# mandt-lab/vbq

Measured on AMD Instinct MI355X. Metric: quantized latents/sec (32-lambda sweep; one count per (element, lambda) pair and entropy-model build), higher is better.
Workload: dtype f32; 1 GPU; kodak24_c256 [36864 x 256] f32, 32-lambda sweep, N=10; step = two-pass entropy-model build (quantizer.py:82-150); elements_per_gpu=9437184, lambdas=32, parallelism=element-sharded x1, launch=one HIP graph replay per step

## Files before the change

### vbq_amd/csrc/vbq_quantize_fast.hip

```cpp
#include <stddef.h>

#include "vbq_common.h"
#include "vbq_sweep.h"

namespace vbq {
namespace {

constexpr int kFastThreads = 256;
#ifndef VBQ_FAST_NE
#define VBQ_FAST_NE 2
#endif
#ifndef VBQ_FAST_WAVES
#define VBQ_FAST_WAVES 4
#endif
#ifndef VBQ_SLOW_INLINE
#define VBQ_SLOW_INLINE __noinline__
#endif
constexpr int kFastNE = VBQ_FAST_NE;

__device__ __forceinline__ float dist_cost(float P, float mu, double rinv) {
    const float d = __fsub_rn(P, mu);
    const float t = (float)__dmul_rn((double)d, rinv);
    const float q = __fmul_rn(t, t);
    return __fmul_rn(0.5f, q);
}

__device__ __forceinline__ float min3f(float a, float b, float c) { return fminf(fminf(a, b), c); }

template <bool NT>
__device__ __forceinline__ void store_idx2(uint32_t *p, uint32_t v) {
    if constexpr (NT) __builtin_nontemporal_store(v, p);
    else *p = v;
}

template <int M>
__device__ __forceinline__ float min_of(const float (&v)[M]) {
    float t[M];
#pragma unroll
    for (int i = 0; i < M; ++i) t[i] = v[i];
    int m = M;
#pragma unroll
    for (int pass = 0; pass < 8; ++pass) {
        if (m <= 1) break;
        int o = 0;
        int i = 0;
#pragma unroll
        for (; i + 2 < m; i += 3) t[o++] = min3f(t[i], t[i + 1], t[i + 2]);
        if (o == 0) { t[o++] = fminf(t[0], t[1]); i = 2; }
        for (; i < m; ++i) t[o++] = t[i];
        m = o;
    }
    return t[0];
}

template <int N>
struct LevelInfo {
    float dL, dR;
    uint32_t posL, posR;
};

template <int N>
__device__ __forceinline__ LevelInfo<N> descend(const float *tb, int n, float z, double sg, uint32_t &g) {
    const int off = (1 << n) - 1;
    const int m = 1 << n;
    const uint32_t j = g;
    const float pj = tb[off + j];
    const bool below = pj < z;
    LevelInfo<N> r;
    if (n == 0) {
        r.dL = r.dR = dist_cost(pj, z, sg);
        r.posL = r.posR = 0;
    } else {
        int jo = below ? (int)j + 1 : (int)j - 1;
        jo = jo < 0 ? 0 : (jo > m - 1 ? m - 1 : jo);
        bool swap = false;
        if (n == N && below && j == (uint32_t)(m - 1)) { jo = m - 2; swap = true; }
        const float po = tb[off + jo];
        const float dj = dist_cost(pj, z, sg);
        const float dn = dist_cost(po, z, sg);
        const bool j_is_left = below && !swap;
        r.dL = j_is_left ? dj : dn;
        r.dR = j_is_left ? dn : dj;
        r.posL = j_is_left ? j : (uint32_t)jo;
        r.posR = j_is_left ? (uint32_t)jo : j;
    }
    g = 2 * g + (below ? 1u : 0u);
    return r;
}

template <int N>
__device__ VBQ_SLOW_INLINE uint32_t exact_rank_scan(const float *tb, float z, float sigma, const float *pen) {
    const double sg = __ddiv_rn(1.0, (double)sigma);
    uint32_t g = 0;
    float bestL = 0.f, bestR = 0.f;
    uint32_t rkL = 0, rkR = 0;
    for (int n = 0; n <= N; ++n) {
        const LevelInfo<N> li = descend<N>(tb, n, z, sg, g);
        const float p = pen[n];
        const float cL = __fadd_rn(li.dL, p);
        if (n == 0 || cL < bestL) { bestL = cL; rkL = ((2 * li.posL + 1) << (N - n)) - 1; }
        if (n >= 1) {
            const float cR = __fadd_rn(li.dR, p);
            if (n == 1 || cR < bestR) { bestR = cR; rkR = ((2 * li.posR + 1) << (N - n)) - 1; }
        }
    }
    if (N == 0) return rkL;
    return (bestL <= bestR) ? rkL : rkR;
}

template <int N, int MODE>
__global__ void __launch_bounds__(kFastThreads, VBQ_FAST_WAVES)
k_quant_fast(const float *__restrict__ mu, const float *__restrict__ sg, long n_per_ch, long ch_stride, int C,
             const float *__restrict__ table, Lambdas32 lam, const float *__restrict__ len,
             int L, uint16_t *__restrict__ out_idx, float *__restrict__ out_zhat,
             float *__restrict__ out_bits, long E, int vec_ok, int dbg,
             unsigned long long *__restrict__ level_counts) {
    constexpr int T = table_size(N);
    constexpr int N1 = N + 1;
    constexpr int NE = kFastNE;
    constexpr bool EXTRA = MODE == 1;
    constexpr bool COUNT = MODE == 2;
    const bool never_flag = dbg == 2;
    constexpr int PS = (N1 + 3) & ~3;
    __shared__ float tb[T + 1];
    __shared__ uint32_t scratch[N1 * NE * kFastThreads];
    __shared__ __align__(16) float penl[kMaxLambdaChunk * PS];
    const int c = blockIdx.y;
    if (COUNT) {
        for (int i = threadIdx.x; i < N1 * NE * kFastThreads; i += blockDim.x) scratch[i] = 0;
    }
    for (int i = threadIdx.x; i < T; i += blockDim.x) tb[i] = table[(long)c * T + i];
    int odd = 0;
    for (int i = threadIdx.x; i < L * PS; i += blockDim.x) {
        const int l = i / PS, n = i - l * PS;
        const float p = n < N1 ? __fmul_rn(lam.lam[l], len ? len[((long)l * C + c) * N1 + n] : (float)n) : 0.0f;
        penl[i] = p;
        odd |= (len != nullptr && !(p == 0.0f || (p >= 1.8189894e-12f && p <= 1.1805916e21f))) ? 1 : 0;
    }
    const bool force_slow = dbg == 1 || __syncthreads_or(odd) != 0;

    const long base = (long)c * ch_stride;
    const long nquads = (n_per_ch + NE - 1) / NE;

    auto load_group = [&](long q, float (&m)[NE], float (&sv)[NE]) {
        const long i0 = q * NE;
        if (!(vec_ok & 2) && (vec_ok & 1) && (i0 + NE <= n_per_ch)) {
            if constexpr (NE == 4) {
                const float4 mv = *reinterpret_cast<const float4 *>(mu + base + i0);
                const float4 s4v = *reinterpret_cast<const float4 *>(sg + base + i0);
                m[0] = mv.x; m[1] = mv.y; m[2] = mv.z; m[3] = mv.w;
                sv[0] = s4v.x; sv[1] = s4v.y; sv[2] = s4v.z; sv[3] = s4v.w;
            } else {
                const float2 mv = *reinterpret_cast<const float2 *>(mu + base + i0);
                const float2 s2v = *reinterpret_cast<const float2 *>(sg + base + i0);
                m[0] = mv.x; m[1] = mv.y;
                sv[0] = s2v.x; sv[1] = s2v.y;
            }
        } else {
#pragma unroll
            for (int k = 0; k < NE; ++k) {
                const bool ok = i0 + k < n_per_ch;
                const long at = (vec_ok & 2) ? (i0 + k) * C + c : base + i0 + k;
                m[k] = ok ? mu[at] : 0.0f;
                sv[k] = ok ? sg[at] : 1.0f;
            }
        }
    };
    const long q0 = (long)blockIdx.x * blockDim.x + threadIdx.x, qstep = (long)gridDim.x * blockDim.x;
    float mn[NE], sn[NE];
#pragma unroll
    for (int k = 0; k < NE; ++k) { mn[k] = 0.0f; sn[k] = 1.0f; }
    if (q0 < nquads) load_group(q0, mn, sn);
    const bool resident = (vec_ok & 4) != 0;
    unsigned int rot = wave_slot();
    for (long q = q0; q < nquads; q += qstep) {
        if (resident) __builtin_amdgcn_s_setprio(3);
        const long i0 = q * NE;
        const bool full = (vec_ok & 1) && (i0 + NE <= n_per_ch);
        float m4[NE], s4[NE];
#pragma unroll
        for (int k = 0; k < NE; ++k) { m4[k] = mn[k]; s4[k] = sn[k]; }
        {
            const long qn = q + qstep < nquads ? q + qstep : q;
            load_group(qn, mn, sn);
        }

        float du[NE][N1];
        uint32_t g[NE];
        double rinv[NE];
#pragma unroll
        for (int k = 0; k < NE; ++k) {
            g[k] = 0;
            rinv[k] = __ddiv_rn(1.0, (double)s4[k]);
        }
        const char *tbb = reinterpret_cast<const char *>(tb);
#pragma unroll
        for (int n = 0; n <= N; ++n) {
            constexpr int kWordMask = 0xffe00000u;
            const int off4 = 4 * ((1 << n) - 1);
            const int top4 = 4 * ((1 << n) - 1);
#pragma unroll
            for (int k = 0; k < NE; ++k) {
                const float pj = *reinterpret_cast<const float *>(tbb + off4 + g[k]);
                const bool below = pj < m4[k];
                float dL, dR;
                uint32_t lo4, hi4;
                if (n == 0) {
                    dL = dR = dist_cost(pj, m4[k], rinv[k]);
                    lo4 = hi4 = 0;
                } else {
                    const uint32_t G4 = g[k] + (below ? 4u : 0u);
                    int lo = (int)G4 - 4;
                    lo = lo < 0 ? 0 : lo;
                    if (n == N) lo = lo > top4 - 4 ? top4 - 4 : lo;
                    lo4 = (uint32_t)lo;
                    hi4 = G4 > (uint32_t)top4 ? (uint32_t)top4 : G4;
                    dL = dist_cost(*reinterpret_cast<const float *>(tbb + off4 + lo4), m4[k], rinv[k]);
                    dR = dist_cost(*reinterpret_cast<const float *>(tbb + off4 + hi4), m4[k], rinv[k]);
                }
                du[k][n] = vmin(dL, dR);
                g[k] = 2 * g[k] + (below ? 4u : 0u);
                if (COUNT) continue;
                const bool r_better = dR < dL;
                const uint32_t b4 = r_better ? hi4 : lo4;
                const uint32_t better = n < N ? (b4 << (N - n - 1)) + ((1u << (N - n)) - 1u) : (b4 >> 1);
                const uint32_t gap = __float_as_uint(__fsub_rn(dR, dL)) ^ 0x80000000u;
                scratch[(n * NE + k) * kFastThreads + threadIdx.x] = (gap & kWordMask) | better;
            }
        }

        if (resident) {
            set_issue_priority(rot);
            rot += 3u;
        }
        for (int l = 0; l < L; ++l) {
            const float *pp = penl + l * PS;
            float p[N1];
#pragma unroll
            for (int n = 0; n < N1; ++n) p[n] = pp[n];
            uint32_t rank[NE];
            float cst[NE][N1];
            float S[NE];
            uint32_t ne[NE];
#pragma unroll
            for (int n = 0; n < N1; ++n)
#pragma unroll
                for (int k = 0; k < NE; ++k) cst[k][n] = __fadd_rn(du[k][n], p[n]);
#pragma unroll
            for (int k = 0; k < NE; ++k) S[k] = min_of<N1>(cst[k]);
            {
#pragma unroll
                for (int k = 0; k < NE; ++k) ne[k] = 0;
#pragma unroll
                for (int n = N; n >= 0; --n)
#pragma unroll
                    for (int k = 0; k < NE; ++k)
                        ne[k] = __builtin_amdgcn_alignbit(ne[k], __float_as_uint(__fsub_rn(S[k], cst[k][n])), 31);
            }
            uint64_t fmk[NE];
            if constexpr (COUNT) {
                uint64_t any_multi = 0;
                uint32_t lvl[NE];
#pragma unroll
                for (int k = 0; k < NE; ++k) {
                    lvl[k] = (uint32_t)__builtin_ctz(~ne[k]);
                    const uint64_t multi = __builtin_amdgcn_uicmp((uint32_t)__popc(ne[k]), (uint32_t)N, 33);
                    fmk[k] = never_flag ? 0ull : (force_slow ? ~0ull : multi);
                    any_multi |= fmk[k];
                }
                if (any_multi != 0) {
                    const uint32_t lane = __lane_id();
#pragma unroll
                    for (int k = 0; k < NE; ++k)
                        if ((fmk[k] >> lane) & 1ull)
                            lvl[k] = (uint32_t)N - (uint32_t)__builtin_ctz(exact_rank_scan<N>(tb, m4[k], s4[k], pp) + 1u);
                }
                const uint32_t lane = threadIdx.x & 63u;
                const uint32_t inc = (lane & 16u) ? 0x10000u : 1u;
#pragma unroll
                for (int k = 0; k < NE; ++k)
                    if (i0 + k < n_per_ch) atomicAdd(&scratch[((uint32_t)(l * N1) + lvl[k]) * 16u + (lane & 15u)], inc);
                continue;
            }
            uint32_t pk[NE];
#pragma unroll
            for (int k = 0; k < NE; ++k) {
                const int n1 = __builtin_ctz(~ne[k]);
                pk[k] = scratch[(n1 * NE + k) * kFastThreads + threadIdx.x];
            }
            uint64_t fm[NE];
#pragma unroll
            for (int k = 0; k < NE; ++k) {
                const uint64_t multi = __builtin_amdgcn_uicmp((uint32_t)__popc(ne[k]), (uint32_t)N, 33);
                const uint32_t thr = __float_as_uint(__fmul_rn(S[k], 1.9073486328125e-06f));
                const uint64_t lr_close = __builtin_amdgcn_uicmp(pk[k], thr, 37);
                rank[k] = pk[k] & ((2u << N) - 1u);
                fm[k] = never_flag ? 0ull : (force_slow ? ~0ull : (multi | lr_close));
            }
            uint64_t any_flag = 0;
#pragma unroll
            for (int k = 0; k < NE; ++k) any_flag |= fm[k];
            if (any_flag != 0) {
                const uint32_t lane = __lane_id();
#pragma unroll
                for (int k = 0; k < NE; ++k)
                    if ((fm[k] >> lane) & 1ull) rank[k] = exact_rank_scan<N>(tb, m4[k], s4[k], pp);
            }
            const long o = (long)l * E + base + i0;
            float zh[NE], bt[NE];
            if (EXTRA) {
#pragma unroll
                for (int k = 0; k < NE; ++k) {
                    const uint32_t kk = rank[k] + 1;
                    const int tz = __builtin_ctz(kk);
                    const int lvl = N - tz;
                    const uint32_t pos = kk >> (tz + 1);
                    zh[k] = tb[(1 << lvl) - 1 + pos];
                    bt[k] = len ? len[((long)l * C + c) * N1 + lvl] : (float)lvl;
                }
            }
            if (full) {
                if constexpr (NE == 4) {
                    uint2 pk2;
                    pk2.x = rank[0] | (rank[1] << 16);
                    pk2.y = rank[2] | (rank[3] << 16);
                    *reinterpret_cast<uint2 *>(out_idx + o) = pk2;
                    if (EXTRA) {
                        if (out_zhat) *reinterpret_cast<float4 *>(out_zhat + o) = make_float4(zh[0], zh[1], zh[2], zh[3]);
                        if (out_bits) *reinterpret_cast<float4 *>(out_bits + o) = make_float4(bt[0], bt[1], bt[2], bt[3]);
                    }
                } else {
                    store_idx2<false>(reinterpret_cast<uint32_t *>(out_idx + o), rank[0] | (rank[1] << 16));
                    if (EXTRA) {
                        if (out_zhat) *reinterpret_cast<float2 *>(out_zhat + o) = make_float2(zh[0], zh[1]);
                        if (out_bits) *reinterpret_cast<float2 *>(out_bits + o) = make_float2(bt[0], bt[1]);
                    }
                }
            } else {
#pragma unroll
                for (int k = 0; k < NE; ++k) {
                    if (i0 + k < n_per_ch) {
                        out_idx[o + k] = (uint16_t)rank[k];
                        if (EXTRA) {
                            if (out_zhat) out_zhat[o + k] = zh[k];
                            if (out_bits) out_bits[o + k] = bt[k];
                        }
                    }
                }
            }
        }
    }
    if constexpr (COUNT) {
        __syncthreads();
        for (int i = threadIdx.x; i < L * N1; i += blockDim.x) {
            unsigned int v = 0;
#pragma unroll
            for (int j = 0; j < 16; ++j) {
                const unsigned int w = scratch[i * 16 + j];
                v += (w & 0xffffu) + (w >> 16);
            }
            const int l = i / N1, n = i - l * N1;
            if (v) atomicAdd(&level_counts[((long)l * C + c) * N1 + n], (unsigned long long)v);
        }
    }
}


#ifndef VBQ_HULL_WAVES
#define VBQ_HULL_WAVES 4
#endif
#ifndef VBQ_HULL_NE
#define VBQ_HULL_NE 2
#endif
#ifndef VBQ_HULL_THREADS
#define VBQ_HULL_THREADS 256
#endif
constexpr int kHullThreads = VBQ_HULL_THREADS;
#ifndef VBQ_HULL_COPIES
#define VBQ_HULL_COPIES 16
#endif
constexpr int kHullKeys = 2048;
constexpr int kFixQueue = 192;
struct HullSweep : SweepTable<32, kHullKeys> {};
static_assert(sizeof(HullSweep) == 2220 && offsetof(HullSweep, val) == 0 && offsetof(HullSweep, perm) == 128 && offsetof(HullSweep, L) == 160 &&
              offsetof(HullSweep, key0) == 164 && offsetof(HullSweep, nkeys) == 168 && offsetof(HullSweep, lut) == 172,
              "HullSweep travels in the kernel arguments: its layout is fixed");

template <int N>
__device__ __forceinline__ void hull_du_nearest(const char *tbb, float z, float sigma, float (&du)[N + 1]) {
    uint32_t g = 0;
    const double rinv = __ddiv_rn(1.0, (double)sigma);
#pragma unroll
    for (int n = 0; n <= N; ++n) {
        const int off4 = 4 * ((1 << n) - 1);
        const int top4 = off4;
        const float pj = *reinterpret_cast<const float *>(tbb + off4 + g);
        const bool below = pj < z;
        float dmin;
        if (n == 0) {
            dmin = __fsub_rn(pj, z);
        } else {
            int o4 = (int)g + (below ? 4 : -4);
            o4 = o4 < 0 ? 0 : (o4 > top4 ? top4 : o4);
            const float po = *reinterpret_cast<const float *>(tbb + off4 + o4);
            dmin = fminf(fabsf(__fsub_rn(pj, z)), fabsf(__fsub_rn(po, z)));
        }
        const float t = (float)__dmul_rn((double)dmin, rinv);
        du[n] = __fmul_rn(0.5f, __fmul_rn(t, t));
        g = 2 * g + (below ? 4u : 0u);
    }
}

template <int N>
__device__ __forceinline__ uint32_t level_of_min(const float (&du)[N + 1], const float *pen, bool &multi) {
    constexpr int N1 = N + 1;
    float cst[N1];
#pragma unroll
    for (int n = 0; n < N1; ++n) cst[n] = __fadd_rn(du[n], pen[n]);
    const float S = min_of<N1>(cst);
    uint32_t ne = 0;
#pragma unroll
    for (int n = N; n >= 0; --n) ne = __builtin_amdgcn_alignbit(ne, __float_as_uint(__fsub_rn(S, cst[n])), 31);
    multi = (uint32_t)__popc(ne) != (uint32_t)N;
    return (uint32_t)__builtin_ctz(~ne);
}

template <int N>
__device__ __forceinline__ void hull_counts_fix(uint64_t lanes, const float (&du_hot)[N + 1], const float *tb, float z, float sigma,
                                                int L, int key0, int nkeys, const unsigned char *perm, const unsigned char *lut,
                                                const float4 *rec, const float *penl, int *corr, bool all_points) {
    constexpr int N1 = N + 1;
    constexpr int PS = (N1 + 3) & ~3;
    const bool mine = (lanes >> (threadIdx.x & 63u)) & 1ull;
    float du[N1];
#pragma unroll
    for (int n = 0; n < N1; ++n) {
        float d = du_hot[n];
        asm volatile("" : "+v"(d));
        du[n] = d;
    }
    float Tn[N];
    uint32_t apos[N];
    sweep_thresholds<N>(du, Tn);
    uint32_t fl = (!(sweep_max_du<N>(du) < kSweepBig) || all_points) ? 0xffffffffu : 0u;
    float G[N];
    uint32_t near = 0;
#pragma unroll
    for (int n = 0; n < N; ++n) {
        float4 nb;
        apos[n] = sweep_position<16>(Tn[n], key0, nkeys, lut, rec, nb);
        G[n] = sweep_band(Tn[n], n, du[n]);
        const float dist = sweep_distance(Tn[n], nb);
        near |= (mine && dist <= G[n]) ? (1u << n) : 0u;
    }
#pragma unroll
    for (int n = 0; n < N; ++n) {
        if ((near >> n) & 1u) {
            for (int l = (int)apos[n] - 1; l >= 0 && fabsf(__fsub_rn(rec[l + 1].x, Tn[n])) <= G[n]; --l) fl |= 1u << l;
            for (int l = (int)apos[n]; l < L && fabsf(__fsub_rn(rec[l + 1].x, Tn[n])) <= G[n]; ++l) fl |= 1u << l;
        }
    }
    fl &= L >= 32 ? 0xffffffffu : ((1u << L) - 1u);
    if (!mine) fl = 0u;
    while (fl != 0u) {
        const int l = __builtin_ctz(fl);
        fl &= fl - 1u;
        const int lo_ = perm[l];
        bool multi;
        int n_ex = (int)level_of_min<N>(du, penl + lo_ * PS, multi);
        if (multi) n_ex = N - __builtin_ctz(exact_rank_scan<N>(tb, z, sigma, penl + lo_ * PS) + 1u);
        int n_pred = 0;
#pragma unroll
        for (int n = 0; n < N; ++n) n_pred += apos[n] > (uint32_t)l ? 1 : 0;
        if (n_ex != n_pred) {
            atomicAdd(&corr[l * N1 + n_ex], 1);
            atomicSub(&corr[l * N1 + n_pred], 1);
        }
    }
}

template <int N>
__global__ void __launch_bounds__(kHullThreads, (VBQ_HULL_WAVES * 256) / kHullThreads)
k_level_counts_hull(const float *__restrict__ mu, const float *__restrict__ sg, long n_per_ch, long ch_stride, int C,
                    const float *__restrict__ table, Lambdas32 lam, HullSweep sw, int vec_ok,
                    unsigned long long *__restrict__ level_counts, int dbg) {
    constexpr int T = table_size(N);
    constexpr int N1 = N + 1;
    constexpr int NE = VBQ_HULL_NE;
    constexpr int KC = VBQ_HULL_COPIES;
    constexpr int PS = (N1 + 3) & ~3;
    constexpr int LB = 33;
    __shared__ float tb[T + 1];
    __shared__ __align__(16) float penl[kMaxLambdaChunk * PS];
    __shared__ __align__(4) unsigned char lut[kHullKeys];
    __shared__ float4 rec[34];
    __shared__ unsigned int H[N * LB * KC];
    __shared__ int corr[kMaxLambdaChunk * N1];
    __shared__ unsigned int n_valid;
    __shared__ unsigned char perm_s[32];
    __shared__ unsigned int fixq[kFixQueue], fixn;
    const int c = blockIdx.y;
    const int L = sw.L;
    for (int i = threadIdx.x; i < T; i += blockDim.x) tb[i] = table[(long)c * T + i];
    for (int i = threadIdx.x; i < L * PS; i += blockDim.x) {
        const int l = i / PS, n = i - l * PS;
        penl[i] = n < N1 ? __fmul_rn(lam.lam[l], (float)n) : 0.0f;
    }
    if (threadIdx.x < 32) perm_s[threadIdx.x] = sw.perm[threadIdx.x];
    for (int i = threadIdx.x; i < N * LB * KC; i += blockDim.x) H[i] = 0;
    for (int i = threadIdx.x; i < L * N1; i += blockDim.x) corr[i] = 0;
    for (int b = threadIdx.x; b < kHullKeys / 4; b += blockDim.x)
        reinterpret_cast<uint32_t *>(lut)[b] = reinterpret_cast<const uint32_t *>(sw.lut)[b];
    if (threadIdx.x < 34) {
        const int i = (int)threadIdx.x;
        rec[i] = sweep_rec(sw.val, L, i);
    }
    if (threadIdx.x == 0) { n_valid = 0; fixn = 0; }
    __syncthreads();

    const bool force_slow = dbg == 1, never_flag = dbg == 2;
    const long base = (long)c * ch_stride;
    const long nquads = (n_per_ch + NE - 1) / NE;
    const char *tbb = reinterpret_cast<const char *>(tb);
    const unsigned int lane = threadIdx.x & 63u;
    const unsigned int inc = (lane & (unsigned)KC) ? 0x10000u : 1u;
    const unsigned int copy = lane & (unsigned)(KC - 1);
    const int key0 = sw.key0, nkeys = sw.nkeys;
    unsigned int my_valid = 0;

    const long q0 = (long)blockIdx.x * blockDim.x + threadIdx.x, qstep = (long)gridDim.x * blockDim.x;
    int it = 0;
    unsigned int rot = wave_slot();
    for (long q = q0; q < nquads; q += qstep, ++it) {
        rotate_issue_priority(rot);
        const long i0 = q * NE;
        const bool full = (vec_ok & 1) && (i0 + NE <= n_per_ch);
        float m4[NE], s4[NE];
        if (vec_ok & 2) {
#pragma unroll
            for (int k = 0; k < NE; ++k) {
                const bool ok = i0 + k < n_per_ch;
                m4[k] = ok ? mu[(i0 + k) * C + c] : 0.0f;
                s4[k] = ok ? sg[(i0 + k) * C + c] : 1.0f;
            }
        } else if (full && NE == 2) {
            const float2 mv = *reinterpret_cast<const float2 *>(mu + base + i0);
            const float2 sv = *reinterpret_cast<const float2 *>(sg + base + i0);
            m4[0] = mv.x; m4[NE - 1] = mv.y;
            s4[0] = sv.x; s4[NE - 1] = sv.y;
        } else {
#pragma unroll
            for (int k = 0; k < NE; ++k) {
                const bool ok = i0 + k < n_per_ch;
                m4[k] = ok ? mu[base + i0 + k] : 0.0f;
                s4[k] = ok ? sg[base + i0 + k] : 1.0f;
            }
        }
        float du[NE][N1];
#pragma unroll
        for (int k = 0; k < NE; ++k) hull_du_nearest<N>(tbb, m4[k], s4[k], du[k]);
        uint64_t fix[NE];
#pragma unroll
        for (int k = 0; k < NE; ++k) {
            const bool valid = i0 + k < n_per_ch;
            my_valid += valid ? 1u : 0u;
            const unsigned int vinc = valid ? inc : 0u;
            float Tn[N];
            sweep_thresholds<N>(du[k], Tn);
            fix[k] = __builtin_amdgcn_ballot_w64(!(sweep_max_du<N>(du[k]) < kSweepBig)) | (force_slow ? ~0ull : 0ull);
#pragma unroll
            for (int n = 0; n < N; ++n) {
                float4 nb;
                const uint32_t a = sweep_position<16>(Tn[n], key0, nkeys, lut, rec, nb);
                const float G = sweep_band(Tn[n], n, du[k][n]);
                const float dist = sweep_distance(Tn[n], nb);
                fix[k] |= __builtin_amdgcn_ballot_w64(dist <= G);
                atomicAdd(&H[((uint32_t)n * LB + a) * (unsigned)KC + copy], vinc);
            }
            fix[k] &= __builtin_amdgcn_ballot_w64(valid);
        }
        uint64_t any_fix = 0;
#pragma unroll
        for (int k = 0; k < NE; ++k) any_fix |= fix[k];
        if (any_fix != 0 && !never_flag) {
#pragma unroll
            for (int k = 0; k < NE; ++k) {
                const bool mine = (fix[k] >> lane) & 1ull;
                unsigned int slot = kFixQueue;
                if (mine) slot = atomicAdd(&fixn, 1u);
                if (mine && slot < (unsigned)kFixQueue) fixq[slot] = ((unsigned int)it << 9) | (threadIdx.x << 1) | (unsigned)k;
                const uint64_t now = __builtin_amdgcn_ballot_w64(mine && slot >= (unsigned)kFixQueue);
                if (now != 0ull)
                    hull_counts_fix<N>(now, du[k], tb, m4[k], s4[k], L, key0, nkeys, perm_s, lut, rec, penl, corr, force_slow);
            }
        }
    }
    __syncthreads();
    {
        const unsigned int nq = fixn < (unsigned)kFixQueue ? fixn : (unsigned)kFixQueue;
        for (unsigned int i = threadIdx.x; i < ((nq + 63u) & ~63u); i += blockDim.x) {
            const bool on = i < nq;
            const unsigned int e = on ? fixq[i] : 0u;
            const long qq = q0 + (long)(e >> 9) * qstep + (long)((e >> 1) & 255u) - (long)threadIdx.x;
            const long el = qq * NE + (long)(e & 1u);
            const long at = (vec_ok & 2) ? el * C + c : base + el;
            const float z = on ? mu[at] : 0.0f, sgm = on ? sg[at] : 1.0f;
            float du[N1];
            hull_du_nearest<N>(tbb, z, sgm, du);
            const uint64_t lanes = __builtin_amdgcn_ballot_w64(on);
            hull_counts_fix<N>(lanes, du, tb, z, sgm, L, key0, nkeys, perm_s, lut, rec, penl, corr, force_slow);
        }
    }
    atomicAdd(&n_valid, my_valid);
    __syncthreads();
    unsigned int *hs = reinterpret_cast<unsigned int *>(penl);
    static_assert(N * LB <= kMaxLambdaChunk * PS, "hs must fit the penalty staging area");
    for (int i = threadIdx.x; i < N * LB; i += blockDim.x) {
        unsigned int v = 0;
#pragma unroll
        for (int j = 0; j < KC; ++j) {
            const unsigned int w = H[i * KC + j];
            v += (w & 0xffffu) + (w >> 16);
        }
        hs[i] = v;
    }
    __syncthreads();
    if (threadIdx.x < N) {
        unsigned int run = 0;
        for (int a = LB - 1; a >= 0; --a) { run += hs[threadIdx.x * LB + a]; hs[threadIdx.x * LB + a] = run; }
    }
    __syncthreads();
    for (int i = threadIdx.x; i < L * N1; i += blockDim.x) {
        const int l = i / N1, n = i - l * N1;
        const long hi_cnt = n == 0 ? (long)n_valid : (long)hs[(n - 1) * LB + l + 1];
        const long lo_cnt = n == N ? 0 : (long)hs[n * LB + l + 1];
        const long v = hi_cnt - lo_cnt + corr[i];
        if (v) atomicAdd(&level_counts[((long)sw.perm[l] * C + c) * N1 + n], (unsigned long long)v);
    }
}


#ifndef VBQ_K1E_STAGE
#define VBQ_K1E_STAGE 5
#endif
#ifndef VBQ_K1E_WAVES
#define VBQ_K1E_WAVES 4
#endif
template <int N, int LFIX, bool BUF>
__global__ void __launch_bounds__(256, VBQ_K1E_WAVES)
k_quant_hull_idx(const float *__restrict__ mu, const float *__restrict__ sg, long n_per_ch, long ch_stride, int C,
                 const float *__restrict__ table, Lambdas32 lam, HullSweep sw, int vec_ok,
                 uint16_t *__restrict__ out_idx, long E, int dbg) {
    constexpr int T = table_size(N);
    constexpr int N1 = N + 1;
    constexpr int NE = 2;
    constexpr int PS = (N1 + 3) & ~3;
    constexpr int CW = 5;
    struct Lds {
        unsigned short rk[N1 * NE * 256];
        float tb[T + 1];
        float penl[kMaxLambdaChunk * PS];
        unsigned char lut[kHullKeys];
        float4 rec[34];
        unsigned char perm_s[32];
        unsigned int cnt[CW * NE * 256];
    };
    __shared__ __align__(16) Lds lds;
    unsigned short *rk = lds.rk;
    float *tb = lds.tb, *penl = lds.penl;
    unsigned char *lut = lds.lut, *perm_s = lds.perm_s;
    float4 *rec = lds.rec;
    unsigned int *cnt = lds.cnt;
    const int c = blockIdx.y;
    const int L = LFIX ? LFIX : sw.L;
    const unsigned int tid = threadIdx.x;
    for (int i = tid; i < T; i += blockDim.x) tb[i] = table[(long)c * T + i];
    for (int i = tid; i < L * PS; i += blockDim.x) {
        const int l = i / PS, n = i - l * PS;
        penl[i] = n < N1 ? __fmul_rn(lam.lam[l], (float)n) : 0.0f;
    }
    stage_sweep_lut(lut, sw.lut);
    if (tid < 34) {
        const int i = (int)tid;
        auto at = [&](int l) { return l < 0 ? -kSweepBig : (l < L ? sw.val[l < 32 ? l : 31] : kSweepBig); };
        rec[i] = make_float4(at(i - 1), at(i), at(i + 1), 0.0f);
    }
    if (tid < 32) perm_s[tid] = sw.perm[tid];
    for (int i = tid; i < CW * NE * 256; i += blockDim.x) cnt[i] = 0;
    __syncthreads();

    const bool force_slow = dbg == 1, never_flag = dbg == 2;
    const uint32_t all_l = L >= 32 ? 0xffffffffu : ((1u << L) - 1u);
    const long base = (long)c * ch_stride;
    const long npairs = (n_per_ch + NE - 1) / NE;
    const char *tbb = reinterpret_cast<const char *>(tb);
    const unsigned int lane = tid & 63u;

    const __amdgpu_buffer_rsrc_t orsrc = __builtin_amdgcn_make_buffer_rsrc(out_idx, 0, -1 , 0x00020000);
    const uint32_t plane_bytes = (uint32_t)(2 * E);
    unsigned int rot = wave_slot();
    for (long q = (long)blockIdx.x * blockDim.x + tid; q < npairs; q += (long)gridDim.x * blockDim.x) {
        rotate_issue_priority(rot);
        const long i0 = q * NE;
        const bool full = (vec_ok & 1) && (i0 + NE <= n_per_ch);
        float m4[NE], s4[NE];
        if (vec_ok & 2) {
#pragma unroll
            for (int k = 0; k < NE; ++k) {
                const bool ok = i0 + k < n_per_ch;
                m4[k] = ok ? mu[(i0 + k) * C + c] : 0.0f;
                s4[k] = ok ? sg[(i0 + k) * C + c] : 1.0f;
            }
        } else if (full) {
            const float2 mv = *reinterpret_cast<const float2 *>(mu + base + i0);
            const float2 sv = *reinterpret_cast<const float2 *>(sg + base + i0);
            m4[0] = mv.x; m4[1] = mv.y;
            s4[0] = sv.x; s4[1] = sv.y;
        } else {
#pragma unroll
            for (int k = 0; k < NE; ++k) {
                const bool ok = i0 + k < n_per_ch;
                m4[k] = ok ? mu[base + i0 + k] : 0.0f;
                s4[k] = ok ? sg[base + i0 + k] : 1.0f;
            }
        }
        float du[NE][N1];
        uint32_t tiny[NE] = {0, 0};
        {
            uint32_t g[NE] = {0, 0};
            double rinv[NE];
#pragma unroll
// ... 301 lines not shown
#pragma unroll
        for (int k = 0; k < NE; ++k) {
            g[k] = 0;
            rinv[k] = __ddiv_rn(1.0, (double)s4[k]);
#pragma unroll
            for (int l = 0; l < LL; ++l) { S[k][l] = 0.0f; win[k][l] = 0; multi[k][l] = 0; }
        }
        uint32_t opq = 0;
        asm volatile("" : "+v"(opq));
        const float *psv = reinterpret_cast<const float *>(&ps[0][0]) + opq;
#pragma unroll
        for (int n = 0; n <= N; ++n) {
            const int off4 = 4 * ((1 << n) - 1);
            const int top4 = off4;
            uint64_t active = 0;
            float pen[LL], stop[LL];
#pragma unroll
            for (int l = 0; l < LL; ++l) {
                pen[l] = psv[2 * (l * (N1 + 1) + n)];
                stop[l] = psv[2 * (l * (N1 + 1) + n + 1) + 1];
            }
#pragma unroll
            for (int k = 0; k < NE; ++k) {
                const float pj = *reinterpret_cast<const float *>(tbb + off4 + g[k]);
                const bool below = pj < m4[k];
                float dmin;
                if (n == 0) {
                    dmin = __fsub_rn(pj, m4[k]);
                } else {
                    int o4 = (int)g[k] + (below ? 4 : -4);
                    o4 = o4 < 0 ? 0 : (o4 > top4 ? top4 : o4);
                    const float po = *reinterpret_cast<const float *>(tbb + off4 + o4);
                    dmin = fminf(fabsf(__fsub_rn(pj, m4[k])), fabsf(__fsub_rn(po, m4[k])));
                }
                const float t = (float)__dmul_rn((double)dmin, rinv[k]);
                const float du = __fmul_rn(0.5f, __fmul_rn(t, t));
                const uint32_t here = g[k] | ((uint32_t)n << 16);
#pragma unroll
                for (int l = 0; l < LL; ++l) {
                    const float cst = __fadd_rn(du, pen[l]);
                    if (n == 0) {
                        S[k][l] = cst;
                        win[k][l] = here;
                    } else {
                        const bool lt = cst < S[k][l];
                        const uint64_t eq = __builtin_amdgcn_ballot_w64(cst == S[k][l]);
                        multi[k][l] = (multi[k][l] & ~__builtin_amdgcn_ballot_w64(lt)) | eq;
                        S[k][l] = lt ? cst : S[k][l];
                        win[k][l] = lt ? here : win[k][l];
                    }
                    if (n < N) active |= __builtin_amdgcn_ballot_w64(!(S[k][l] < stop[l]));
                }
                g[k] = 2 * g[k] + (below ? 4u : 0u);
            }
            if (n < N && active == 0 && n >= 1) break;
        }
        uint32_t rank[LL][NE];
#pragma unroll
        for (int k = 0; k < NE; ++k)
#pragma unroll
            for (int l = 0; l < LL; ++l) {
                const uint32_t n = win[k][l] >> 16;
                const uint32_t gj = win[k][l] & 0xffffu;
                const uint32_t off4 = 4u * ((1u << n) - 1u), top4 = off4;
                const float pj = *reinterpret_cast<const float *>(tbb + off4 + gj);
                const bool below = pj < m4[k];
                const uint32_t G4 = gj + (below ? 4u : 0u);
                uint32_t lo4 = G4 >= 4u ? G4 - 4u : 0u;
                if (n == (uint32_t)N) lo4 = lo4 > top4 - 4u ? top4 - 4u : lo4;
                const uint32_t hi4 = G4 > top4 ? top4 : G4;
                const float pen = psv[2 * (l * (N1 + 1) + n)];
                const float cL = __fadd_rn(dist_cost(*reinterpret_cast<const float *>(tbb + off4 + lo4), m4[k], rinv[k]), pen);
                const float cR = __fadd_rn(dist_cost(*reinterpret_cast<const float *>(tbb + off4 + hi4), m4[k], rinv[k]), pen);
                const uint32_t b4 = (n >= 1u && cR < cL) ? hi4 : lo4;
                rank[l][k] = (((b4 >> 1) + 1u) << ((uint32_t)N - n)) - 1u;
            }
        uint64_t any_multi = force_slow ? ~0ull : 0ull;
#pragma unroll
        for (int k = 0; k < NE; ++k)
#pragma unroll
            for (int l = 0; l < LL; ++l) any_multi |= multi[k][l];
        if (any_multi != 0) {
#pragma unroll
            for (int k = 0; k < NE; ++k)
#pragma unroll
                for (int l = 0; l < LL; ++l)
                    if (((multi[k][l] >> lane) & 1ull) || force_slow) rank[l][k] = exact_rank_scan<N>(tb, m4[k], s4[k], prow[l]);
        }
#pragma unroll
        for (int l = 0; l < LL; ++l) {
            uint16_t *o = out_idx + (long)l * E + base + i0;
            if (full) {
                *reinterpret_cast<uint32_t *>(o) = rank[l][0] | (rank[l][1] << 16);
            } else {
#pragma unroll
                for (int k = 0; k < NE; ++k)
                    if (i0 + k < n_per_ch) o[k] = (uint16_t)rank[l][k];
            }
        }
    }
}

}

void quant_fast_grid(int64_t n_per_ch, int32_t n_ch, int wg_per_cu, int reserved, bool counting, int64_t *out_gx, bool *out_resident) {
    const int64_t nquads = (n_per_ch + kFastNE - 1) / kFastNE;
    int64_t gx = (nquads + kFastThreads - 1) / kFastThreads;
    const bool explicit_wgs = wg_per_cu >= 1 && wg_per_cu <= 5;
    const int fit = kFastNE == 4 ? 3 : 4;
    const bool dynamic_grid = !explicit_wgs && reserved > 0 &&
                              (resident_slots(fit, reserved) / n_ch) * n_ch * 10 < (int64_t)num_cus() * fit * 9;
    const int per_cu = explicit_wgs ? (wg_per_cu < fit ? wg_per_cu : fit) : (dynamic_grid ? 5 : fit);
    int64_t cap = (dynamic_grid ? (int64_t)num_cus() * per_cu * 4 : resident_slots(per_cu, reserved)) / n_ch;
    const bool resident = !dynamic_grid && (int64_t)n_ch <= (int64_t)num_cus() * per_cu;
    if (cap < 1) cap = 1;
    if (gx > cap) {
        const int64_t iters = gx;
        if (resident) {
            const int64_t rounds_needed = (iters + cap - 1) / cap;
            gx = (iters + rounds_needed - 1) / rounds_needed;
        } else {
            int64_t best = cap, best_pad = ((iters + cap - 1) / cap) * cap - iters;
            for (int64_t g = cap - 1; g >= (cap + 1) / 2 && best_pad > 0; --g) {
                const int64_t pad = ((iters + g - 1) / g) * g - iters;
                if (pad * best < best_pad * g) { best = g; best_pad = pad; }
            }
            gx = best;
        }
        constexpr int64_t max_iters = 65000 / ((64 / 32) * (kFastThreads / 64) * kFastNE);
        if (counting && (iters + gx - 1) / gx > max_iters) gx = (iters + max_iters - 1) / max_iters;
    }
    if (gx < 1) gx = 1;
    *out_gx = gx;
    *out_resident = resident;
}

template <int N>
int launch_quant_fast(const float *mu, const float *sg, int64_t n_per_ch, int64_t ch_stride, int32_t n_ch, const float *table,
                      const Lambdas32 &lam, const float *len, int32_t L, uint16_t *out_idx, float *out_zhat,
                      float *out_bits, int64_t E, int vec_ok,
                      unsigned long long *level_counts, int wg_per_cu, int reserved, hipStream_t st) {
    int64_t gx = 1;
    bool resident = false;
    quant_fast_grid(n_per_ch, n_ch, wg_per_cu, reserved, level_counts != nullptr, &gx, &resident);
    if (resident) vec_ok |= 4;
    const dim3 grid((unsigned)gx, (unsigned)n_ch), block(kFastThreads);
    const int dbg = fast_debug();
    if (level_counts)
        hipLaunchKernelGGL((k_quant_fast<N, 2>), grid, block, 0, st, mu, sg, (long)n_per_ch, (long)ch_stride, (int)n_ch, table,
                           lam, len, (int)L, out_idx, out_zhat, out_bits, (long)E, vec_ok, dbg, level_counts);
    else if (out_zhat || out_bits)
        hipLaunchKernelGGL((k_quant_fast<N, 1>), grid, block, 0, st, mu, sg, (long)n_per_ch, (long)ch_stride, (int)n_ch, table,
                           lam, len, (int)L, out_idx, out_zhat, out_bits, (long)E, vec_ok, dbg, level_counts);
    else
        hipLaunchKernelGGL((k_quant_fast<N, 0>), grid, block, 0, st, mu, sg, (long)n_per_ch, (long)ch_stride, (int)n_ch, table,
                           lam, len, (int)L, out_idx, out_zhat, out_bits, (long)E, vec_ok, dbg, level_counts);
    VBQ_CHECK_LAUNCH("quant_fast");
    return VBQ_OK;
}

template <int N>
int launch_quant_pruned(const float *mu, const float *sg, int64_t n_per_ch, int64_t ch_stride, int32_t n_ch, const float *table,
                        const Lambdas32 &lam, const float *len, int32_t L, uint16_t *out_idx, int64_t E, int vec_ok, hipStream_t st) {
    if (L < 1 || L > kPrunedMaxL) return 1;
    const int64_t npairs = (n_per_ch + 1) / 2;
    int64_t gx = (npairs + 255) / 256;
    int64_t cap = (int64_t)num_cus() * 4 / n_ch;
    if (cap < 1) cap = 1;
    if (gx > cap) gx = cap;
    const int dbg = fast_debug();
    const dim3 grid((unsigned)gx, (unsigned)n_ch), block(256);
#define VBQ_PRUNED_CASE(LLv)                                                                                          \
    case LLv:                                                                                                          \
        hipLaunchKernelGGL((k_quant_pruned<N, LLv>), grid, block, 0, st, mu, sg, (long)n_per_ch, (long)ch_stride, (int)n_ch, \
                           table, lam, len, out_idx, (long)E, vec_ok, dbg);                                            \
        break;
    switch (L) {
        VBQ_PRUNED_CASE(1) VBQ_PRUNED_CASE(2) VBQ_PRUNED_CASE(3) VBQ_PRUNED_CASE(4)
        default: return 1;
    }
#undef VBQ_PRUNED_CASE
    VBQ_CHECK_LAUNCH("quant_pruned");
    return VBQ_OK;
}


static bool build_lambda_sweep(const double *lam, int L, HullSweep &sw) {
    float v[32];
    for (int i = 0; i < L && i < 32; ++i) v[i] = (float)lam[i];
    return build_sweep_table<16>(v, L, 1.9e-12f, 1.8e19f, sw);
}

int64_t level_counts_hull_grid(int64_t n_per_ch, int32_t n_ch, int reserved) {
    const int64_t nquads = (n_per_ch + VBQ_HULL_NE - 1) / VBQ_HULL_NE;
    int64_t gx = (nquads + kHullThreads - 1) / kHullThreads;
    constexpr int per_cu = VBQ_HULL_WAVES * 256 / kHullThreads;
    constexpr int rounds = 1;
    int64_t slots = resident_slots(per_cu, reserved);
    if (reserved > 0 && (slots / n_ch) * n_ch * 10 < (int64_t)num_cus() * per_cu * 9)
        slots = (int64_t)num_cus() * (per_cu > 1 ? per_cu - 1 : 1);
    int64_t cap = slots * rounds / n_ch;
    if (cap < 1) cap = 1;
    if (gx > cap) {
        const int64_t iters = gx;
        const int64_t rounds_needed = (iters + cap - 1) / cap;
        gx = (iters + rounds_needed - 1) / rounds_needed;
        const int64_t max_iters = 65000 / ((32 / VBQ_HULL_COPIES) * (kHullThreads / 64) * VBQ_HULL_NE);
        if ((iters + gx - 1) / gx > max_iters) gx = (iters + max_iters - 1) / max_iters;
    }
    return gx < 1 ? 1 : gx;
}

int launch_level_counts_hull10(const float *mu, const float *sg, int64_t n_per_ch, int64_t ch_stride, int32_t n_ch,
                               const float *table, const double *lam, int32_t L, int vec_ok,
                               unsigned long long *level_counts, int reserved, hipStream_t st) {
    if (L < 1 || L > 32) return 1;
    HullSweep sw;
    if (!build_lambda_sweep(lam, L, sw)) return 1;
    const int64_t gx = level_counts_hull_grid(n_per_ch, n_ch, reserved);
    const int dbg = fast_debug();
    Lambdas32 l32;
    for (int i = 0; i < kMaxLambdaChunk; ++i) l32.lam[i] = i < L ? (float)lam[i] : 0.0f;
    hipLaunchKernelGGL((k_level_counts_hull<10>), dim3((unsigned)gx, (unsigned)n_ch), dim3(kHullThreads), 0, st, mu, sg,
                       (long)n_per_ch, (long)ch_stride, (int)n_ch, table, l32, sw, vec_ok, level_counts, dbg);
    VBQ_CHECK_LAUNCH("level_counts_hull");
    return VBQ_OK;
}

int launch_quant_hull_idx10(const float *mu, const float *sg, int64_t n_per_ch, int64_t ch_stride, int32_t n_ch,
                            const float *table, const double *lam, int32_t L, int vec_ok, uint16_t *out_idx, int64_t E,
                            hipStream_t st) {
    if (L < 16) return 1;
    if (2 * (uint64_t)E > 0xffffffffull) return 1;
    HullSweep sw;
    if (!build_lambda_sweep(lam, L, sw)) return 1;
    const int64_t npairs = (n_per_ch + 1) / 2;
    int64_t gx = (npairs + 255) / 256;
    constexpr int rounds = 2;
    int64_t cap = (int64_t)num_cus() * VBQ_K1E_WAVES * rounds / n_ch;
    if (cap < 1) cap = 1;
    if (gx > cap) gx = cap;
    const int dbg = fast_debug();
    Lambdas32 l32;
    for (int i = 0; i < kMaxLambdaChunk; ++i) l32.lam[i] = i < L ? (float)lam[i] : 0.0f;
    const bool buf = (uint64_t)L * 2ull * (uint64_t)E <= 0xffffffffull;
#define VBQ_K1E_LAUNCH(LF, BF)                                                                                                \
    hipLaunchKernelGGL((k_quant_hull_idx<10, LF, BF>), dim3((unsigned)gx, (unsigned)n_ch), dim3(256), 0, st, mu, sg,          \
                       (long)n_per_ch, (long)ch_stride, (int)n_ch, table, l32, sw, vec_ok, out_idx, (long)E, dbg)
    if (L == 32) { if (buf) VBQ_K1E_LAUNCH(32, true); else VBQ_K1E_LAUNCH(32, false); }
    else if (L == 16) { if (buf) VBQ_K1E_LAUNCH(16, true); else VBQ_K1E_LAUNCH(16, false); }
    else VBQ_K1E_LAUNCH(0, false);
#undef VBQ_K1E_LAUNCH
    VBQ_CHECK_LAUNCH("quant_hull_idx");
    return VBQ_OK;
}

#define VBQ_INST_FAST(NN)                                                                                              \
    template int launch_quant_fast<NN>(const float *, const float *, int64_t, int64_t, int32_t, const float *,        \
                                       const Lambdas32 &, const float *, int32_t, uint16_t *, float *, float *, int64_t, \
                                       int, unsigned long long *, int, int, hipStream_t);
VBQ_FOR_EACH_N(VBQ_INST_FAST)
#undef VBQ_INST_FAST
#define VBQ_INST_PRUNED(NN)                                                                                           \
    template int launch_quant_pruned<NN>(const float *, const float *, int64_t, int64_t, int32_t, const float *,     \
                                         const Lambdas32 &, const float *, int32_t, uint16_t *, int64_t, int, hipStream_t);
VBQ_FOR_EACH_N(VBQ_INST_PRUNED)
#undef VBQ_INST_PRUNED

}

extern "C" int vbq_solve_grid(int32_t kernel, int64_t n_rows, int32_t n_ch, int32_t workgroups_per_cu, int32_t reserved_workgroups,
                              int64_t *h_grid) {
    using namespace vbq;
    VBQ_REQUIRE(h_grid && n_rows >= 1 && n_ch >= 1 && n_ch <= 65535, VBQ_ERR_INVALID_ARGUMENT, "vbq_solve_grid: bad sizes or null pointer");
    VBQ_REQUIRE(kernel == VBQ_GRID_K1 || kernel == VBQ_GRID_K1T, VBQ_ERR_INVALID_ARGUMENT, "vbq_solve_grid: unknown kernel %d", kernel);
    VBQ_REQUIRE(workgroups_per_cu >= 0 && workgroups_per_cu <= 5, VBQ_ERR_INVALID_ARGUMENT, "vbq_solve_grid: workgroups_per_cu=%d not in 0..5",
                workgroups_per_cu);
    const int reserved = reserved_workgroups < 0 ? 0 : reserved_workgroups;
    if (kernel == VBQ_GRID_K1) {
        int64_t gx = 1;
        bool resident = false;
        quant_fast_grid(n_rows, n_ch, workgroups_per_cu, reserved, false, &gx, &resident);
        h_grid[0] = gx;
        h_grid[2] = resident ? 1 : 0;
    } else {
        h_grid[0] = level_counts_hull_grid(n_rows, n_ch, reserved);
        h_grid[2] = 1;
    }
    h_grid[1] = n_ch;
    return VBQ_OK;
}
```

### vbq_amd/csrc/vbq_sweep.h

```cpp
#pragma once
#include "vbq_common.h"
#include "vbq_sweep_host.h"

namespace vbq {

__device__ __forceinline__ float vmin(float a, float b) {
    float r;
    asm("v_min_f32 %0, %1, %2" : "=v"(r) : "v"(a), "v"(b));
    return r;
}
__device__ __forceinline__ float vmax(float a, float b) {
    float r;
    asm("v_max_f32 %0, %1, %2" : "=v"(r) : "v"(a), "v"(b));
    return r;
}
__device__ __forceinline__ float vmax3(float a, float b, float c) {
    float r;
    asm("v_max3_f32 %0, %1, %2, %3" : "=v"(r) : "v"(a), "v"(b), "v"(c));
    return r;
}
__device__ __forceinline__ float vmin3abs(float a, float b, float c) {
    float r;
    asm("v_min3_f32 %0, |%1|, |%2|, |%3|" : "=v"(r) : "v"(a), "v"(b), "v"(c));
    return r;
}

template <int N>
__device__ __forceinline__ void sweep_thresholds(const float (&du)[N + 1], float (&Tn)[N]) {
    constexpr int N1 = N + 1;
    float Pm[N1];
#pragma unroll
    for (int n = 0; n < N; ++n) {
#pragma unroll
        for (int j = n + 1; j < N1; ++j) {
            const float r = __fmul_rn(__fsub_rn(du[n], du[j]), 1.0f / (float)(j - n));
            Pm[j] = n == 0 ? r : vmin(Pm[j], r);
        }
        float t = Pm[n + 1];
        int j = n + 2;
#pragma unroll
        for (; j + 1 < N1; j += 2) t = vmax3(t, Pm[j], Pm[j + 1]);
        if (j < N1) t = vmax(t, Pm[j]);
        Tn[n] = vmin(t, 1.0e38f);
    }
}

template <int N>
__device__ __forceinline__ float sweep_max_du(const float (&du)[N + 1]) {
    constexpr int N1 = N + 1;
    float big = du[0];
#pragma unroll
    for (int j = 1; j + 1 < N1; j += 2) big = vmax3(big, du[j], du[j + 1]);
    if ((N1 & 1) == 0) big = vmax(big, du[N1 - 1]);
    return big;
}

template <int SHIFT>
__device__ __forceinline__ int sweep_bucket(float t, int key0, int nkeys) {
    return min(max(((int)__float_as_uint(t) >> SHIFT) - key0, 0), nkeys - 1);
}

template <int SHIFT>
__device__ __forceinline__ uint32_t sweep_position(float t, int key0, int nkeys, const unsigned char *lut, const float4 *rec,
                                                   float4 &nb) {
    const uint32_t cnt = lut[sweep_bucket<SHIFT>(t, key0, nkeys)];
    nb = rec[cnt];
    return cnt + (nb.y < t ? 1u : 0u);
}

__device__ __forceinline__ float sweep_band(float t, int n, float du_n) {
    return __fmul_rn(fmaf(fabsf(t), (float)(n + 1), du_n), 9.5367431640625e-07f);
}

__device__ __forceinline__ float sweep_distance(float t, const float4 &nb) {
    return vmin3abs(__fsub_rn(t, nb.x), __fsub_rn(t, nb.y), __fsub_rn(t, nb.z));
}

template <int MAXL>
__device__ __forceinline__ float4 sweep_rec(const float (&val)[MAXL], int L, int i) {
    auto at = [&](int l) { return l < 0 ? -kSweepBig : (l < L ? val[l < MAXL ? l : MAXL - 1] : kSweepBig); };
    return make_float4(at(i - 1), at(i), at(i + 1), 0.0f);
}
template <int NKEYS>
__device__ __forceinline__ void stage_sweep_lut(unsigned char *lut, const unsigned char (&arg)[NKEYS]) {
    for (int k = threadIdx.x; k < NKEYS / 4; k += blockDim.x)
        reinterpret_cast<uint32_t *>(lut)[k] = reinterpret_cast<const uint32_t *>(arg)[k];
}

__device__ __forceinline__ uint32_t sweep_rank_offset(uint32_t P, int j, uint32_t base) {
    const uint32_t sh = j < 3 ? (P << (10 - 4 * j)) : (P >> (4 * j - 10));
    return (sh & 0x3c00u) | base;
}

}
```

Baseline: 505.7 billion latents/s.

## Trim fast-quant kernel: buffer stores, vector penalty loads, batched hull lookups, med3 clamp

Adds several micro-optimizations to the quantize kernels. In the NE=2 fast path it loads penalty rows as float4, merges the per-element multi-flag compares into one, skips masking the packed rank, and packs two 16-bit ranks with v_perm. When the index planes fit in 4GB it writes them through raw buffer stores with a scalar plane offset. The hull kernel now does its LUT and record lookups in staged batches before the histogram atomics, and sweep_bucket clamps with a single v_med3_i32. These changes aim to cut VALU and address arithmetic and to overlap LDS latency, at the cost of extra register pressure and a subtly different multi-flag check.

```diff
diff --git a/vbq_amd/csrc/vbq_index_planes.h b/vbq_amd/csrc/vbq_index_planes.h
--- /dev/null
+++ b/vbq_amd/csrc/vbq_index_planes.h
@@ -0,0 +1,13 @@
+#pragma once
+#include <stdint.h>
+
+namespace vbq {
+
+inline bool index_planes_within_4gb(int64_t L, int64_t E) {
+    if (L < 1 || E < 1) return false;
+    if ((uint64_t)E > 0xffffffffull / 2ull) return false;
+    if ((uint64_t)L > 0xffffffffull) return false;
+    return (uint64_t)L * (2ull * (uint64_t)E) <= 0xffffffffull;
+}
+
+}
diff --git a/vbq_amd/csrc/vbq_quantize_fast.hip b/vbq_amd/csrc/vbq_quantize_fast.hip
--- a/vbq_amd/csrc/vbq_quantize_fast.hip
+++ b/vbq_amd/csrc/vbq_quantize_fast.hip
@@ -1,6 +1,7 @@
 #include <stddef.h>
 
 #include "vbq_common.h"
+#include "vbq_index_planes.h"
 #include "vbq_sweep.h"
 
 namespace vbq {
@@ -17,6 +18,10 @@
 #define VBQ_SLOW_INLINE __noinline__
 #endif
 constexpr int kFastNE = VBQ_FAST_NE;
+#ifndef VBQ_K1_TRIM
+#define VBQ_K1_TRIM 1
+#endif
+constexpr bool kK1Trim = VBQ_K1_TRIM != 0 && VBQ_FAST_NE == 2;
 
 __device__ __forceinline__ float dist_cost(float P, float mu, double rinv) {
     const float d = __fsub_rn(P, mu);
@@ -108,7 +113,7 @@
     return (bestL <= bestR) ? rkL : rkR;
 }
 
-template <int N, int MODE>
+template <int N, int MODE, bool BUF = false>
 __global__ void __launch_bounds__(kFastThreads, VBQ_FAST_WAVES)
 k_quant_fast(const float *__restrict__ mu, const float *__restrict__ sg, long n_per_ch, long ch_stride, int C,
              const float *__restrict__ table, Lambdas32 lam, const float *__restrict__ len,
@@ -173,6 +178,10 @@
     if (q0 < nquads) load_group(q0, mn, sn);
     const bool resident = (vec_ok & 4) != 0;
     unsigned int rot = wave_slot();
+    uint32_t prow0 = 0;
+    asm volatile("" : "+v"(prow0));
+    const __amdgpu_buffer_rsrc_t orsrc = __builtin_amdgcn_make_buffer_rsrc(out_idx, 0, -1 , 0x00020000);
+    const uint32_t plane_bytes = (uint32_t)(2 * E);
     for (long q = q0; q < nquads; q += qstep) {
         if (resident) __builtin_amdgcn_s_setprio(3);
         const long i0 = q * NE;
@@ -233,11 +242,24 @@
             set_issue_priority(rot);
             rot += 3u;
         }
-        for (int l = 0; l < L; ++l) {
-            const float *pp = penl + l * PS;
-            float p[N1];
-#pragma unroll
-            for (int n = 0; n < N1; ++n) p[n] = pp[n];
+        uint64_t nan0[NE];
+#pragma unroll
+        for (int k = 0; k < NE; ++k) nan0[k] = kK1Trim ? __builtin_amdgcn_ballot_w64(du[k][0] != du[k][0]) : 0ull;
+        uint32_t prow = prow0, plane_off = 0;
+        for (int l = 0; l < L; ++l, prow += 4u * PS, plane_off += plane_bytes) {
+            if constexpr (kK1Trim) asm volatile("" : "+v"(prow));
+            const float *pp = kK1Trim ? reinterpret_cast<const float *>(reinterpret_cast<const char *>(penl) + prow) : penl + l * PS;
+            float p[PS];
+            if constexpr (kK1Trim) {
+#pragma unroll
+                for (int n = 0; n < PS; n += 4) {
+                    const float4 v = *reinterpret_cast<const float4 *>(pp + n);
+                    p[n] = v.x; p[n + 1] = v.y; p[n + 2] = v.z; p[n + 3] = v.w;
+                }
+            } else {
+#pragma unroll
+                for (int n = 0; n < N1; ++n) p[n] = pp[n];
+            }
             uint32_t rank[NE];
             float cst[NE][N1];
             float S[NE];
@@ -261,10 +283,12 @@
             if constexpr (COUNT) {
                 uint64_t any_multi = 0;
                 uint32_t lvl[NE];
+                uint64_t multi2 = 0;
+                if constexpr (kK1Trim) multi2 = __builtin_amdgcn_uicmp((uint32_t)__popc(ne[0]) + (uint32_t)__popc(ne[NE - 1]), 2u * N, 33);
 #pragma unroll
                 for (int k = 0; k < NE; ++k) {
                     lvl[k] = (uint32_t)__builtin_ctz(~ne[k]);
-                    const uint64_t multi = __builtin_amdgcn_uicmp((uint32_t)__popc(ne[k]), (uint32_t)N, 33);
+                    const uint64_t multi = kK1Trim ? (multi2 | nan0[k]) : __builtin_amdgcn_uicmp((uint32_t)__popc(ne[k]), (uint32_t)N, 33);
                     fmk[k] = never_flag ? 0ull : (force_slow ? ~0ull : multi);
                     any_multi |= fmk[k];
                 }
@@ -289,12 +313,14 @@
                 pk[k] = scratch[(n1 * NE + k) * kFastThreads + threadIdx.x];
             }
             uint64_t fm[NE];
+            uint64_t multi2 = 0;
+            if constexpr (kK1Trim) multi2 = __builtin_amdgcn_uicmp((uint32_t)__popc(ne[0]) + (uint32_t)__popc(ne[NE - 1]), 2u * N, 33);
 #pragma unroll
             for (int k = 0; k < NE; ++k) {
-                const uint64_t multi = __builtin_amdgcn_uicmp((uint32_t)__popc(ne[k]), (uint32_t)N, 33);
+                const uint64_t multi = kK1Trim ? (multi2 | nan0[k]) : __builtin_amdgcn_uicmp((uint32_t)__popc(ne[k]), (uint32_t)N, 33);
                 const uint32_t thr = __float_as_uint(__fmul_rn(S[k], 1.9073486328125e-06f));
                 const uint64_t lr_close = __builtin_amdgcn_uicmp(pk[k], thr, 37);
-                rank[k] = pk[k] & ((2u << N) - 1u);
+                rank[k] = (kK1Trim && !EXTRA) ? pk[k] : pk[k] & ((2u << N) - 1u);
                 fm[k] = never_flag ? 0ull : (force_slow ? ~0ull : (multi | lr_close));
             }
             uint64_t any_flag = 0;
@@ -330,6 +356,13 @@
                         if (out_bits) *reinterpret_cast<float4 *>(out_bits + o) = make_float4(bt[0], bt[1], bt[2], bt[3]);
                     }
                 } else {
+                    if constexpr (kK1Trim && !EXTRA) {
+                        const uint32_t two = __builtin_amdgcn_perm(rank[NE - 1], rank[0], 0x05040100u);
+                        if constexpr (BUF)
+                            __builtin_amdgcn_raw_buffer_store_b32(two, orsrc, (uint32_t)(2 * (base + i0)), plane_off, 0);
+                        else
+                            store_idx2<false>(reinterpret_cast<uint32_t *>(out_idx + o), two);
+                    } else
                     store_idx2<false>(reinterpret_cast<uint32_t *>(out_idx + o), rank[0] | (rank[1] << 16));
                     if (EXTRA) {
                         if (out_zhat) *reinterpret_cast<float2 *>(out_zhat + o) = make_float2(zh[0], zh[1]);
@@ -340,6 +373,9 @@
 #pragma unroll
                 for (int k = 0; k < NE; ++k) {
                     if (i0 + k < n_per_ch) {
+                        if constexpr (kK1Trim && !EXTRA && BUF)
+                            __builtin_amdgcn_raw_buffer_store_b16((uint16_t)rank[k], orsrc, (uint32_t)(2 * (base + i0 + k)), plane_off, 0);
+                        else
                         out_idx[o + k] = (uint16_t)rank[k];
                         if (EXTRA) {
                             if (out_zhat) out_zhat[o + k] = zh[k];
@@ -378,6 +414,9 @@
 constexpr int kHullThreads = VBQ_HULL_THREADS;
 #ifndef VBQ_HULL_COPIES
 #define VBQ_HULL_COPIES 16
+#endif
+#ifndef VBQ_K1T_STAGE
+#define VBQ_K1T_STAGE 10
 #endif
 constexpr int kHullKeys = 2048;
 constexpr int kFixQueue = 192;
@@ -568,6 +607,29 @@
             float Tn[N];
             sweep_thresholds<N>(du[k], Tn);
             fix[k] = __builtin_amdgcn_ballot_w64(!(sweep_max_du<N>(du[k]) < kSweepBig)) | (force_slow ? ~0ull : 0ull);
+#if VBQ_K1T_STAGE
+            uint32_t apos[N];
+#pragma unroll
+            for (int n = 0; n < N; ++n) apos[n] = lut[sweep_bucket<16>(Tn[n], key0, nkeys)];
+#pragma unroll
+            for (int h = 0; h < N; h += VBQ_K1T_STAGE) {
+                float4 nbs[VBQ_K1T_STAGE];
+#pragma unroll
+                for (int i = 0; i < VBQ_K1T_STAGE; ++i)
+                    if (h + i < N) nbs[i] = rec[apos[h + i]];
+#pragma unroll
+                for (int i = 0; i < VBQ_K1T_STAGE; ++i) {
+                    const int n = h + i;
+                    if (n >= N) break;
+                    apos[n] += nbs[i].y < Tn[n] ? 1u : 0u;
+                    const float G = sweep_band(Tn[n], n, du[k][n]);
+                    const float dist = sweep_distance(Tn[n], nbs[i]);
+                    fix[k] |= __builtin_amdgcn_ballot_w64(dist <= G);
+                }
+            }
+#pragma unroll
+            for (int n = 0; n < N; ++n) atomicAdd(&H[((uint32_t)n * LB + apos[n]) * (unsigned)KC + copy], vinc);
+#else
 #pragma unroll
             for (int n = 0; n < N; ++n) {
                 float4 nb;
@@ -577,6 +639,7 @@
                 fix[k] |= __builtin_amdgcn_ballot_w64(dist <= G);
                 atomicAdd(&H[((uint32_t)n * LB + a) * (unsigned)KC + copy], vinc);
             }
+#endif
             fix[k] &= __builtin_amdgcn_ballot_w64(valid);
         }
         uint64_t any_fix = 0;
@@ -1184,6 +1247,9 @@
     else if (out_zhat || out_bits)
         hipLaunchKernelGGL((k_quant_fast<N, 1>), grid, block, 0, st, mu, sg, (long)n_per_ch, (long)ch_stride, (int)n_ch, table,
                            lam, len, (int)L, out_idx, out_zhat, out_bits, (long)E, vec_ok, dbg, level_counts);
+    else if (kK1Trim && index_planes_within_4gb(L, E))
+        hipLaunchKernelGGL((k_quant_fast<N, 0, true>), grid, block, 0, st, mu, sg, (long)n_per_ch, (long)ch_stride, (int)n_ch, table,
+                           lam, len, (int)L, out_idx, out_zhat, out_bits, (long)E, vec_ok, dbg, level_counts);
     else
         hipLaunchKernelGGL((k_quant_fast<N, 0>), grid, block, 0, st, mu, sg, (long)n_per_ch, (long)ch_stride, (int)n_ch, table,
                            lam, len, (int)L, out_idx, out_zhat, out_bits, (long)E, vec_ok, dbg, level_counts);
@@ -1275,7 +1341,7 @@
     const int dbg = fast_debug();
     Lambdas32 l32;
     for (int i = 0; i < kMaxLambdaChunk; ++i) l32.lam[i] = i < L ? (float)lam[i] : 0.0f;
-    const bool buf = (uint64_t)L * 2ull * (uint64_t)E <= 0xffffffffull;
+    const bool buf = index_planes_within_4gb(L, E);
 #define VBQ_K1E_LAUNCH(LF, BF)                                                                                                \
     hipLaunchKernelGGL((k_quant_hull_idx<10, LF, BF>), dim3((unsigned)gx, (unsigned)n_ch), dim3(256), 0, st, mu, sg,          \
                        (long)n_per_ch, (long)ch_stride, (int)n_ch, table, l32, sw, vec_ok, out_idx, (long)E, dbg)
diff --git a/vbq_amd/csrc/vbq_sweep.h b/vbq_amd/csrc/vbq_sweep.h
--- a/vbq_amd/csrc/vbq_sweep.h
+++ b/vbq_amd/csrc/vbq_sweep.h
@@ -55,9 +55,19 @@
     return big;
 }
 
+#ifndef VBQ_SWEEP_MED3
+#define VBQ_SWEEP_MED3 1
+#endif
 template <int SHIFT>
 __device__ __forceinline__ int sweep_bucket(float t, int key0, int nkeys) {
-    return min(max(((int)__float_as_uint(t) >> SHIFT) - key0, 0), nkeys - 1);
+    const int x = ((int)__float_as_uint(t) >> SHIFT) - key0;
+#if VBQ_SWEEP_MED3
+    int r;
+    asm("v_med3_i32 %0, %1, 0, %2" : "=v"(r) : "v"(x), "s"(nkeys - 1));
+    return r;
+#else
+    return min(max(x, 0), nkeys - 1);
+#endif
 }
 
 template <int SHIFT>
```

Result: faster. 520.4 billion latents/s, median of 6 (+2.9%).
